# bonjour-l/esa-pose-estimation

Measured on AMD Instinct MI355X. Metric: HRNet-W32 256x256 crops/sec (heatmaps + fused argmax/refine keypoints), higher is better.
Workload: dtype bf16x6 (fp32-grade: every f32 operand split exactly into 3 bf16 terms, 6 bf16 MFMAs per product, f32 accumulate; f32 NHWC activations; f32 VALU stem conv1 / output layer) — heat-maps closer to fp64 than the fp32 CPU reference; 1 GPU; seg_hrnet2 HRNet-W32 256x256, batch 32/GPU, 11 keypoints, fp32 NCHW in -> heatmaps -> keypoints (BASELINE configs[1]); global_batch=32, per_gpu_batch=32, parallelism=dp1, hip_graph=True

## Files before the change

esa-pose-estimation_amd/csrc/forward.hip:

```cpp
#include <cstdarg>

#include "plan.h"

namespace esa {

__attribute__((format(printf, 3, 4)))
static void describe(esahrnet_op_desc* d, const char* kernel, const char* label, ...) {
    snprintf(d->kernel, sizeof d->kernel, "%s", kernel);
    va_list ap;
    va_start(ap, label);
    vsnprintf(d->label, sizeof d->label, label, ap);
    va_end(ap);
}

Request make_request(Decoder d, void* kp, void* idx, void* hess, void* fit, void* status, void* cov, void* info, double cov_floor,
                     int M, int nms_radius, int refine) {
    Request r;
    r.decoder = d;
    r.kp = static_cast<float*>(kp);
    r.idx = static_cast<int*>(idx);
    r.hess = d == DEC_FINAL ? nullptr : static_cast<double*>(hess);
    r.fit = static_cast<double*>(fit);
    r.status = static_cast<int*>(status);
    r.cov = d == DEC_GAUSSFIT || d == DEC_CAND ? static_cast<double*>(cov) : nullptr;
// ... 357 lines not shown
            p.x0 = T(o.in); p.y = T(o.out);
            p.w0 = static_cast<const uint4*>(c.head_w0); p.w3 = static_cast<const uint4*>(c.head_w3);
            p.bias0 = c.head_b0; p.bias3 = c.head_b3;
            p.N = n; p.H = lh[ti.level]; p.W = lw[ti.level];
            for (int i = 0; i < 3; ++i) {
                const Tensor& tt = c.tensors[o.terms[i]];
                p.t[i] = T(o.terms[i]); p.th[i] = lh[tt.level]; p.tw[i] = lw[tt.level];
                p.Ctp = tt.Cp;
            }
            p.C0p = ti.Cp; p.C3p = to.Cp; p.K = c.cfg.num_keypoints; p.valu = c.opt.bf_head_valu && !c.hf(); p.hf = c.hf();
            if (desc) {
                const ConvSpec& s0 = c.specs[c.spec_l0];
                const ConvSpec& s3 = c.specs[c.spec_l3];
                describe(desc, o.kind == OP_HEAD ? "head_fused" : c.x6() ? "head_x6" : c.hf() ? "head_fused_bf<fp16>" : "head_fused_bf",
                         "last_layer.0[:, 0:%d] + up + last_layer.3", c.head_c0);
                desc->flops = 2.0 * n * lh[to.level] * lw[to.level] * ((double)s0.cout * c.head_c0 + (double)s3.cout * s3.cin);
                desc->bytes = tbytes(o.in) + tbytes(o.out);
                for (int i = 0; i < 3; ++i) desc->bytes += tbytes(o.terms[i]);
            } else if (o.kind == OP_HEADBF) {
                rc = c.x6() ? esa::launch_head_x6(p, stream)
                   : b.h0_rec ? esa::launch_head_bf_range(p, b.h0_part, b.h0_rec, stream) : esa::launch_head_bf(p, stream);
            } else {
                if (!esa::head_fused_supported(p.H, p.W, p.th, p.tw, p.C0p, p.K))
                    return set_error("forward: fused head does not support this shape (%dx%d)", p.H, p.W);
                rc = esa::launch_head(p, stream);
            }
            break;
        }
        case OP_HEADT: {
            const Tensor& ti = c.tensors[o.in];
            const Tensor& to = c.tensors[o.out];
            const DevConv& d = c.dconvs[o.dconv];
            esa::HeadTParams p{};
            p.x = T(o.in); p.t = T(o.out); p.wt = static_cast<const uint4*>(d.w);
            p.N = n; p.h = lh[ti.level]; p.w = lw[ti.level];
            p.Cinp = ti.Cp; p.Ctp = to.Cp; p.XP = esa::head_t_xp(p.w);
            if (desc) {
                const ConvSpec& s = c.specs[d.spec];
                describe(desc, "head_t", "%s[:, %d:%d] (T layout)", s.name.c_str(), d.c0, d.c1);
                desc->flops = 2.0 * n * lh[ti.level] * lw[ti.level] * s.cout * (d.c1 - d.c0);
                desc->bytes = tbytes(o.in) + tbytes(o.out) + (double)esa::packed_weight_bytes(d.coutp, d.cinp, 1);
            } else rc = esa::launch_head_t(p, stream);
            break;
        }
        case OP_HEAD2: {
            const Tensor& ti = c.tensors[o.in];
            const Tensor& to = c.tensors[o.out];
            const DevConv& d1 = c.dconvs[o.dconv];
            esa::Head2Params p{};
            p.x0 = T(o.in); p.x1 = T(o.terms[0]); p.t2 = T(o.terms[1]); p.t3 = T(o.terms[2]); p.y = T(o.out);
            p.w0 = static_cast<const uint4*>(c.head_w0); p.w3 = static_cast<const uint4*>(c.head_w3);
            p.w1 = static_cast<const uint4*>(d1.w);
            p.bias0 = c.head_b0; p.bias3 = c.head_b3;
            p.N = n; p.H = lh[ti.level]; p.W = lw[ti.level];
            for (int i = 0; i < 3; ++i) {
                const Tensor& tt = c.tensors[o.terms[i]];
                p.th[i] = lh[tt.level]; p.tw[i] = lw[tt.level];
            }
            p.xp2 = esa::head_t_xp(p.tw[1]); p.xp3 = esa::head_t_xp(p.tw[2]);
            p.C0p = ti.Cp; p.C1p = c.tensors[o.terms[0]].Cp; p.Ctp = c.tensors[o.terms[1]].Cp;
            p.C3p = to.Cp; p.K = c.cfg.num_keypoints;
            if (desc) {
                const ConvSpec& s0 = c.specs[c.spec_l0];
                const ConvSpec& s3 = c.specs[c.spec_l3];
                const Tensor& t1 = c.tensors[o.terms[0]];
                describe(desc, "head_fused2", "last_layer.0[:, 0:%d] + up (MFMA) + last_layer.3", d1.c1);
                desc->flops = 2.0 * n * lh[to.level] * lw[to.level] * ((double)s0.cout * c.head_c0 + (double)s3.cout * s3.cin) +
                              2.0 * n * lh[t1.level] * lw[t1.level] * (double)s0.cout * (d1.c1 - d1.c0);
                desc->bytes = tbytes(o.in) + tbytes(o.out);
                for (int i = 0; i < 3; ++i) desc->bytes += tbytes(o.terms[i]);
            } else rc = esa::launch_head2(p, sp.head2_ulo, stream);
            break;
        }
        case OP_FUSE: {
            const Tensor& to = c.tensors[o.out];
            esa::FuseParams p{};
            p.nterms = o.nterms;
            for (int i = 0; i < o.nterms; ++i) {
                const Tensor& ti = c.tensors[o.terms[i]];
                if (ti.Cp != to.Cp) return set_error("plan bug: fuse channel mismatch");
                p.x[i] = T(o.terms[i]); p.h[i] = lh[ti.level]; p.w[i] = lw[ti.level];
            }
            p.y = T(o.out); p.N = n; p.H = lh[to.level]; p.W = lw[to.level]; p.Cp = to.Cp;
            p.relu = o.relu; p.fmt = c.opt.fmt;
            if (desc) {
                describe(desc, c.hf() ? "fuse_kernel<fp16>" : "fuse_kernel", "fuse -> %s", to.tap.c_str());
                desc->bytes = tbytes(o.out);
                for (int i = 0; i < o.nterms; ++i) desc->bytes += tbytes(o.terms[i]);
            } else rc = esa::launch_fuse(p, stream);
            break;
        }
        case OP_FINAL: {
            const Tensor& ti = c.tensors[o.in];
            esa::FinalParams p{};
            p.h3 = T(o.in); p.x0 = static_cast<const float*>(b.x); p.out = static_cast<float*>(b.heat);
            p.w = c.final_w; p.bias = c.final_b; p.wpk = static_cast<const uint4*>(c.final_wpk);
            p.N = n; p.H = height; p.W = width; p.h = lh[ti.level]; p.wd = lw[ti.level];
            p.K = c.cfg.num_keypoints; p.cin = c.cfg.cin; p.Cp = ti.Cp; p.fmt = c.opt.fmt;
            p.part = static_cast<float2*>(b.part);
            if (desc) {
                const ConvSpec& s = c.specs[c.spec_final];
                describe(desc, c.hf() ? "final_kernel<fp16>" : "final_kernel", "%s", s.name.c_str());
                desc->flops = 2.0 * n * height * width * s.cout * s.cin * 9;
                desc->bytes = tbytes(o.in) + (double)n * height * width * (c.cfg.cin + s.cout) * 4;
            } else if (b.req.decoder != DEC_NONE)
                rc = run_decode(c, b, &p, nullptr, 0, 0, n, height, width, stream);
            else rc = esa::launch_final(p, stream);
            break;
        }
    }
    if (rc) return set_error("forward: kernel launch failed: %s", hipGetErrorString((hipError_t)rc));
    return 0;
}

int run_forward(esahrnet_handle h, const void* x_dev, int n, int height, int width, void* heat_dev, void* part_dev, void* ws_dev,
                size_t ws_bytes, esahrnet_stream stream_, hipEvent_t* events, const Request* req, void* h0_part, void* h0_rec) {
    if (!h || !x_dev || !(heat_dev || req) || !ws_dev) return set_error("forward: null argument");
    if (!h->committed) return set_error("forward: esahrnet_commit has not been called");
    if (plan_shape(*h, n, height, width)) return 1;
    const KpScratch ks = kp_scratch(*h, n, height, width, req ? req->decoder : DEC_NONE, req ? req->refine : -1);
    if (check_workspace("forward", ws_dev, ws_bytes, h->sp.bytes + ks.total())) return 1;
    hipStream_t stream = static_cast<hipStream_t>(stream_);
    Buffers bufs{x_dev, heat_dev, static_cast<char*>(ws_dev), part_dev};
    bufs.h0_part = h0_part; bufs.h0_rec = h0_rec;
    if (req) {
        char* const scratch = bufs.ws + h->sp.bytes;
        bufs.req = *req;
        bufs.kheat = reinterpret_cast<float*>(scratch);
        bufs.kpart = reinterpret_cast<float2*>(scratch + ks.part_off());
        bufs.kbmax = reinterpret_cast<float*>(scratch + ks.bmax_off());
        bufs.kws = ks.part;
        bufs.kcidx = reinterpret_cast<int*>(scratch + ks.cidx_off());
        bufs.kat = scratch + ks.at_off();
    }
    int op_index = 0;
    if (events && hipEventRecord(events[0], stream) != hipSuccess) return set_error("forward: hipEventRecord failed");
    const bool multi = !events && !h->keep && h->opt.nlanes > 1 && h->side[0] != nullptr;
    const hipStream_t caller = stream;
    bool lane_used[4] = {true, false, false, false};
    int cur_wave = -1;
    auto join = [&](size_t slot, unsigned lanes) -> int {
        for (int l = 1; l < 4; ++l)
            if ((lanes >> l & 1) && lane_used[l]) {
                hipEvent_t e = h->wave_end[slot * 3 + l - 1];
                if (hipEventRecord(e, h->side[l - 1]) != hipSuccess || hipStreamWaitEvent(caller, e, 0) != hipSuccess) return 1;
                lane_used[l] = false;
            }
        return 0;
    };
    for (const Op& o : h->ops) {
        if (multi) {
            if (o.join && join((size_t)op_index, o.join)) return set_error("forward: joining side lanes failed");
            if (o.wave != cur_wave) {
                cur_wave = o.wave;
                if (h->wave_mask[cur_wave] & ~1u) HIP_OK(hipEventRecord(h->wave_entry[cur_wave], caller));
            }
            stream = o.lane == 0 ? caller : h->side[o.lane - 1];
            lane_used[o.lane] = true;
            if (o.wait_entry) HIP_OK(hipStreamWaitEvent(stream, h->wave_entry[cur_wave], 0));
            if (o.wait0 >= 0) HIP_OK(hipStreamWaitEvent(stream, h->op_event[o.wait0], 0));
        }
        if (run_op(*h, o, h->sp, bufs, stream, nullptr)) return 1;
        if (multi && o.record) HIP_OK(hipEventRecord(h->op_event[op_index], caller));
        ++op_index;
        if (events && hipEventRecord(events[op_index], stream) != hipSuccess) return set_error("forward: hipEventRecord failed");
    }
    if (multi && join(h->ops.size(), 0xeu)) return set_error("forward: joining the side lanes failed");
// ... 282 lines not shown
```

esa-pose-estimation_amd/csrc/fuse.hip:

```cpp
#include "kernels.h"
#include "sb.h"

namespace esa {
namespace {

static_assert(FMT_BF == EL_BF && FMT_HF == EL_HF && FMT_SB == EL_SB, "format codes double as element types");

struct Lerp {
    int i0, i1;
    float l0, l1;
};

__device__ __forceinline__ Lerp lerp_ac_false(int dst, int in, int out) {
    const float scale = (float)in / (float)out;
    float src = scale * ((float)dst + 0.5f) - 0.5f;
    src = src < 0.f ? 0.f : src;
    Lerp r;
    r.i0 = min((int)src, in - 1);
    r.i1 = r.i0 + (r.i0 < in - 1 ? 1 : 0);
    r.l1 = src - (float)r.i0;
    r.l0 = 1.f - r.l1;
    return r;
}

// ... 113 lines not shown
            load8<FMT_F32>(p.x[0] + ((row0 + (j >> 1)) * p.W + X + (j & 1)) * (size_t)pixb, c8, acc[j]);
    } else {
#pragma unroll
        for (int j = 0; j < 4; ++j)
#pragma unroll
            for (int i = 0; i < 8; ++i) acc[j][i] = 0.f;
    }
#pragma unroll
    for (int t = 1; t < NS; ++t)
#pragma unroll
        for (int j = 0; j < 4; ++j) {
            float v[8];
            load8<FMT_F32>(p.x[t] + ((row0 + (j >> 1)) * p.W + X + (j & 1)) * (size_t)pixb, c8, v);
#pragma unroll
            for (int i = 0; i < 8; ++i) acc[j][i] += v[i];
        }
#pragma unroll
    for (int k = 0; k < NU; ++k) {
        const int t = NS + k;
        const int h = p.h[t], w = p.w[t];
        const Lerp ly[2] = {lerp_scaled(Y, h, fs.sy[t]), lerp_scaled(Y + 1, h, fs.sy[t])};
        const Lerp lx[2] = {lerp_scaled(X, w, fs.sx[t]), lerp_scaled(X + 1, w, fs.sx[t])};
        const char* base = p.x[t] + (size_t)n * h * w * (size_t)pixb;
        const char* ra = base + (size_t)ly[0].i0 * w * (size_t)pixb;
        const char* rb = base + (size_t)ly[0].i1 * w * (size_t)pixb;
        const char* rc = base + (size_t)ly[1].i1 * w * (size_t)pixb;
        const int ca = lx[0].i0 * pixb, cb = lx[0].i1 * pixb, cc = lx[1].i1 * pixb;
        const bool sely = ly[1].i0 != ly[0].i0, selx = lx[1].i0 != lx[0].i0;
        const bool cell = (cell_mask >> t) & 1;
        if (cell) {
            float v00[8], v01[8], v10[8], v11[8];
            load8<FMT_F32>(ra + ca, c8, v00);
            load8<FMT_F32>(ra + cb, c8, v01);
            load8<FMT_F32>(rb + ca, c8, v10);
            load8<FMT_F32>(rb + cb, c8, v11);
#pragma unroll
            for (int j = 0; j < 4; ++j) {
                const int dy = j >> 1, dx = j & 1;
#pragma unroll
                for (int i = 0; i < 8; ++i)
                    acc[j][i] += ly[dy].l0 * (lx[dx].l0 * v00[i] + lx[dx].l1 * v01[i]) + ly[dy].l1 * (lx[dx].l0 * v10[i] + lx[dx].l1 * v11[i]);
            }
        } else {
            float v[3][3][8];
#pragma unroll
            for (int r = 0; r < 3; ++r) {
                const char* rr = r == 0 ? ra : r == 1 ? rb : rc;
                load8<FMT_F32>(rr + ca, c8, v[r][0]);
                load8<FMT_F32>(rr + cb, c8, v[r][1]);
                load8<FMT_F32>(rr + cc, c8, v[r][2]);
            }
#pragma unroll
            for (int i = 0; i < 8; ++i) {
                float c0[3][2], c1[3][2];
#pragma unroll
                for (int r = 0; r < 3; ++r) {
                    c0[r][0] = v[r][0][i]; c1[r][0] = v[r][1][i];
                    c0[r][1] = selx ? v[r][1][i] : v[r][0][i]; c1[r][1] = v[r][2][i];
                }
#pragma unroll
                for (int dx = 0; dx < 2; ++dx) {
                    const float a0 = lx[dx].l0 * c0[0][dx] + lx[dx].l1 * c1[0][dx];
                    const float b0 = lx[dx].l0 * c0[1][dx] + lx[dx].l1 * c1[1][dx];
                    const float g0 = lx[dx].l0 * c0[2][dx] + lx[dx].l1 * c1[2][dx];
                    acc[dx][i] += ly[0].l0 * a0 + ly[0].l1 * b0;
                    acc[2 + dx][i] += ly[1].l0 * (sely ? b0 : a0) + ly[1].l1 * g0;
                }
            }
        }
        __builtin_amdgcn_sched_barrier(0);
    }
#pragma unroll
    for (int j = 0; j < 4; ++j) {
        if (p.relu) {
#pragma unroll
            for (int i = 0; i < 8; ++i) acc[j][i] = relu1(acc[j][i]);
        }
        char* o = p.y + ((row0 + (j >> 1)) * p.W + X + (j & 1)) * (size_t)pixb + c8 * 32;
        *reinterpret_cast<f32x4*>(o) = f32x4{acc[j][0], acc[j][1], acc[j][2], acc[j][3]};
        *reinterpret_cast<f32x4*>(o + 16) = f32x4{acc[j][4], acc[j][5], acc[j][6], acc[j][7]};
    }
}

template <int NS, int NU>
int launch_fuse_t(const FuseParams& p, const FuseScales& fs, hipStream_t stream) {
    bool blocks = p.fmt == FMT_F32 && NU > 0 && !(p.H & 1) && !(p.W & 1);
    int cell_mask = 0;
    for (int t = NS; t < NS + NU && blocks; ++t) {
        if (2 * p.h[t] > p.H || 2 * p.w[t] > p.W) blocks = false;
        const bool exact = p.h[t] > 0 && p.w[t] > 0 && p.H % p.h[t] == 0 && p.W % p.w[t] == 0;
        const int ry = exact ? p.H / p.h[t] : 0, rx = exact ? p.W / p.w[t] : 0;
        if ((ry == 4 || ry == 8) && (rx == 4 || rx == 8)) cell_mask |= 1 << t;
    }
    if (blocks) {
        const long long per_row = (long long)(p.W >> 1) * (p.Cp >> 3), rows = (long long)p.N * (p.H >> 1);
        if (per_row <= 0 || rows <= 0 || rows > 0x7fffffffLL || per_row > 0x7fffffffLL) return (int)hipErrorInvalidValue;
        hipLaunchKernelGGL((fuse2x2_kernel<NS, NU>), dim3((unsigned)((per_row + 255) / 256), (unsigned)rows), dim3(256), 0, stream, p, fs, cell_mask);
        return (int)hipGetLastError();
    }
    const long long per_row = (long long)p.W * (p.Cp >> 3);
    const long long rows = (long long)p.N * p.H;
    if (per_row <= 0 || rows <= 0 || rows > 0x7fffffffLL || per_row > 0x7fffffffLL) return (int)hipErrorInvalidValue;
    const dim3 grid((unsigned)((per_row + 255) / 256), (unsigned)rows);
    if (p.fmt == FMT_BF) hipLaunchKernelGGL((fuse_kernel<NS, NU, FMT_BF>), grid, dim3(256), 0, stream, p, fs);
    else if (p.fmt == FMT_HF) hipLaunchKernelGGL((fuse_kernel<NS, NU, FMT_HF>), grid, dim3(256), 0, stream, p, fs);
    else if (p.fmt == FMT_F32) hipLaunchKernelGGL((fuse_kernel<NS, NU, FMT_F32>), grid, dim3(256), 0, stream, p, fs);
    else hipLaunchKernelGGL((fuse_kernel<NS, NU, FMT_SB>), grid, dim3(256), 0, stream, p, fs);
    return (int)hipGetLastError();
}

}

int launch_fuse(const FuseParams& p_in, hipStream_t stream) {
    if ((p_in.Cp & 7) || p_in.nterms < 1 || p_in.nterms > 4) return (int)hipErrorInvalidValue;
    FuseParams p = p_in;
    FuseScales fs{};
    int ns = 0, k = 0;
    for (int pass = 0; pass < 2; ++pass)
        for (int t = 0; t < p_in.nterms; ++t) {
            const bool same = p_in.h[t] == p_in.H && p_in.w[t] == p_in.W;
            if (same != (pass == 0)) continue;
            p.x[k] = p_in.x[t]; p.h[k] = p_in.h[t]; p.w[k] = p_in.w[t];
            fs.sy[k] = (float)p_in.h[t] / (float)p_in.H;
            fs.sx[k] = (float)p_in.w[t] / (float)p_in.W;
            ++k;
            if (same) ++ns;
        }
    const int nu = p.nterms - ns;
    switch (ns * 10 + nu) {
        case 1: return launch_fuse_t<0, 1>(p, fs, stream);
        case 2: return launch_fuse_t<0, 2>(p, fs, stream);
        case 3: return launch_fuse_t<0, 3>(p, fs, stream);
        case 4: return launch_fuse_t<0, 4>(p, fs, stream);
        case 10: return launch_fuse_t<1, 0>(p, fs, stream);
        case 11: return launch_fuse_t<1, 1>(p, fs, stream);
        case 12: return launch_fuse_t<1, 2>(p, fs, stream);
        case 13: return launch_fuse_t<1, 3>(p, fs, stream);
        case 20: return launch_fuse_t<2, 0>(p, fs, stream);
        case 21: return launch_fuse_t<2, 1>(p, fs, stream);
        case 22: return launch_fuse_t<2, 2>(p, fs, stream);
        case 30: return launch_fuse_t<3, 0>(p, fs, stream);
        case 31: return launch_fuse_t<3, 1>(p, fs, stream);
        case 40: return launch_fuse_t<4, 0>(p, fs, stream);
    }
    return (int)hipErrorInvalidValue;
}

}
```

esa-pose-estimation_amd/csrc/kernels.h:

```cpp
#pragma once
#include <hip/hip_runtime.h>
#include <stdint.h>

namespace esa {

enum { FMT_SB = 0, FMT_BF = 1, FMT_F32 = 2, FMT_HF = 3 };
inline bool fmt_half(int fmt) { return fmt == FMT_BF || fmt == FMT_HF; }

int set_error(const char* fmt, ...);

struct ConvParams {
    const char* x;
    char* y;
    const char* res;
    const uint4* w;
    const float* bias;
    int N, H, W, OH, OW;
    int Cinp, Coutp;
    int relu;
    int out_f32;
    int fmt;
    int nheads;
    int x6_reload;
    char* yh[3];
// ... 2 lines not shown
};
bool conv_s2c32_multi_supported(const ConvParams& p);
int launch_conv_s2c32_multi(const ConvParams& p, hipStream_t stream);
int launch_conv(const ConvParams& p, int k, int stride, hipStream_t stream);
const char* conv_kernel_name(const ConvParams& p, int k, int stride);
bool conv_s2c32_supported(const ConvParams& p);
int launch_conv_s2c32(const ConvParams& p, hipStream_t stream);
int launch_conv_s1w(const ConvParams& p, hipStream_t stream);
bool conv_is_stream_s1(const ConvParams& p);
bool conv_jobs_supported(const ConvParams* ps, int n, int stride);
int launch_conv_jobs(const ConvParams* ps, int n, int stride, hipStream_t stream);
bool use_th16(const ConvParams& p);
void set_stream_launch_limit(long long bytes);
bool conv1x1_supported(const ConvParams& p);
int launch_conv1x1(const ConvParams& p, hipStream_t stream);
bool conv1x1_jobs_supported(const ConvParams* ps, int n);
int launch_conv1x1_jobs(const ConvParams* ps, int n, hipStream_t stream);
size_t packed_weight_bytes(int coutp, int cinp, int k);
void pack_conv_weights(const float* w, int cout, int cin, int k, int coutp, int cinp, void* dst);
size_t packed_weight_bytes_bf(int coutp, int cinp, int k);
void pack_conv_weights_bf(const float* w, int cout, int cin, int k, int coutp, int cinp, void* dst, bool half = false);
uint16_t host_f16(float f);
bool host_f16_finite(float f);

size_t packed_weight_bytes_x6(int coutp, int cinp, int k);
void pack_conv_weights_x6(const float* w, int cout, int cin, int k, int coutp, int cinp, void* dst);
bool conv_x6_supported(const ConvParams& p, int k, int stride);
int launch_conv_x6(const ConvParams& p, int k, int stride, hipStream_t stream);
const char* conv_x6_kernel_name(const ConvParams& p, int k, int stride);
bool conv_x6_jobs_supported(const ConvParams* ps, int n, int k, int stride);
int launch_conv_x6_jobs(const ConvParams* ps, int n, int k, int stride, hipStream_t stream);
void set_x6_grid_limit(int workgroups);
bool conv1x1_x6_supported(const ConvParams& p);
int launch_conv1x1_x6(const ConvParams& p, hipStream_t stream);
int launch_conv1x1_x6_jobs(const ConvParams* ps, int n, hipStream_t stream);
bool conv1x1_x6_jobs_supported(const ConvParams* ps, int n);

struct StemParams {
    const float* x;
    char* y;
    const float* w;
    const float* bias;
    int N, H, W, cin, cout;
    int relu;
    int fmt;
};
int launch_stem(const StemParams& p, hipStream_t stream);
int stem_pool_slabs(int cin, int cout, int H, int W);
int launch_stem_pool(const StemParams& p, float* pool, hipStream_t stream);

struct BlockParams {
    const char* x;
    char* y;
    const uint4* w1;
    const uint4* w2;
    const float* bias1;
    const float* bias2;
    int N, H, W;
};
int launch_bblock32(const BlockParams& p, hipStream_t stream);

struct StemFusedParams {
    const float* x;
    char* y;
    const float* w1;
    const float* bias1;
    const uint4* w2;
    const float* bias2;
    int N, H, W, OH, OW, cin, Cmid, Coutp;
};
int launch_stem_fused(const StemFusedParams& p, hipStream_t stream);
bool stem_fused_x6_supported(int cin, int cmid, int coutp);
void pack_stem_w1_x6(const float* w, const float* b, float* dst);
int launch_stem_fused_x6(const StemFusedParams& p, hipStream_t stream);

struct FuseParams {
    const char* x[4];
    int h[4], w[4];
    int nterms;
    char* y;
    int N, H, W, Cp;
    int relu;
    int fmt;
};
int launch_fuse(const FuseParams& p, hipStream_t stream);

struct FinalParams {
    const char* h3;
    const float* x0;
    float* out;
    const float* w;
    const float* bias;
    const uint4* wpk;
    int N, H, W, h, wd;
    int K, cin, Cp;
    int fmt;
    float2* part;
};
int launch_final(const FinalParams& p, hipStream_t stream);
int final_kp_tiles(int K, int cin, int H, int W);
int launch_final_kp(const FinalParams& p, float* kp, int* idx_out, hipStream_t stream);
int launch_final_gf(const FinalParams& p, float* kp, int* idx_out, double* fit, int* status, double* hess, hipStream_t stream);
int launch_final_gf_cov(const FinalParams& p, float* kp, int* idx_out, double* fit, int* status, double* hess, double* cov,
                        double* info, double cov_floor, hipStream_t stream);
int final2_valu_tiles(int H, int W);
int launch_final2_kp(const FinalParams& p, float* bmax, float* kp, int* idx_out, hipStream_t stream, double* hess = nullptr);
int final_part_tiles(int K, int cin, int H, int W);
__device__ __forceinline__ void argmax_take(float v, int i, float& bv, int& bi) {
    const bool vn = v != v, bn = bv != bv;
    if (v > bv || (vn && !bn) || ((v == bv || (vn && bn)) && i < bi)) { bv = v; bi = i; }
}
bool final_mfma_supported(int K, int cin);
size_t final_mfma_bytes(int K, int cin);
void pack_final_mfma(const float* w, int K, int cin, void* dst);

struct HeadParams {
    const char* x0;
    const char* t[3];
    char* y;
    const uint4* w0;
    const uint4* w3;
    const float* bias0;
    const float* bias3;
    int N, H, W;
    int th[3], tw[3];
    int C0p, Ctp, C3p, K;
    bool valu;
    bool hf;
};
int launch_head(const HeadParams& p, hipStream_t stream);
bool head_fused_supported(int H, int W, const int th[3], const int tw[3], int C0p, int K);
size_t head_w3_bytes(int K, int Ctp);
void pack_head_w3(const float* w, int K, int Ct, int Ctp, void* dst);
int launch_head_bf(const HeadParams& p, hipStream_t stream);
bool head_fused_bf_supported(int H, int W, const int th[3], const int tw[3], int C0p, int K);
int head_bf_range_tiles(int H, int W);
int launch_head_bf_range(const HeadParams& p, void* part, void* rec, hipStream_t stream);
size_t head_w3_bf_bytes(int K, int Ctp);
void pack_head_w3_bf(const float* w, int K, int Ct, int Ctp, void* dst, bool half = false);

int launch_head_x6(const HeadParams& p, hipStream_t stream);
bool head_x6_supported(int H, int W, const int th[3], const int tw[3], int C0p, int K);

constexpr int HT_PAD = 1;
struct HeadTParams {
    const char* x;
    char* t;
    const uint4* wt;
    int N, h, w, Cinp, Ctp, XP;
};
int launch_head_t(const HeadTParams& p, hipStream_t stream);
int head_t_xp(int w);
bool head_t_supported(int Cinp);
struct Head2Params {
    const char* x0;
    const char* x1;
    const char* t2;
    const char* t3;
    char* y;
    const uint4* w0;
    const uint4* w1;
    const uint4* w3;
    const float* bias0;
    const float* bias3;
    int N, H, W;
    int th[3], tw[3];
// ... 157 lines not shown
```

esa-pose-estimation_amd/csrc/op_abi.hip:

```cpp
#include <algorithm>
#include <cstdint>
#include <cstdio>
#include <cstring>
#include <vector>

#include "../../include/esahrnet.h"
#include "host_util.h"
#include "kernels.h"

using esa::DevScope;
using esa::Format;
using esa::set_error;

static const float* f32(const void* p) { return static_cast<const float*>(p); }
static float* f32(void* p) { return static_cast<float*>(p); }
static bool aligned(const void* p, uintptr_t a) { return (reinterpret_cast<uintptr_t>(p) & (a - 1)) == 0; }

static bool conv_form_ok(int k, int stride) { return (k == 1 && stride == 1) || (k == 3 && (stride == 1 || stride == 2)); }
static bool op_conv_dims_ok(int n, int cin, int cout, int h, int w, int k, int stride) {
    if (n <= 0 || cin <= 0 || cout <= 0 || h <= 0 || w <= 0 || !conv_form_ok(k, stride)) return false;
    return (long long)n * h * w * (long long)((std::max(cin, cout) + 63) & ~63) * 4 <= 0x7fffffffLL;
}
static esa::ConvParams op_conv_shape(const Format& f, int n, int cin, int cout, int h, int w, int stride, int relu, const void* res) {
    esa::ConvParams p{};
    p.N = n; p.H = h; p.W = w; p.OH = stride == 2 ? (h + 1) / 2 : h; p.OW = stride == 2 ? (w + 1) / 2 : w;
    p.Cinp = f.pad(cin); p.Coutp = f.pad(cout); p.relu = relu; p.fmt = f.fmt;
    p.res = static_cast<const char*>(res);
    p.x6_reload = esa::env_on("ESAHRNET_X6_RELOAD_WEIGHTS");
    return p;
}
static int op_conv_device(DevScope& m, const Format& f, esa::ConvParams& p, int cin, int cout, int k, const float* w, const float* b,
                          const void* x_dev, const void* res_dev, int* rc) {
    std::vector<float> bias(p.Coutp, 0.f);
    std::copy(b, b + cout, bias.begin());
    char *xs = nullptr, *rs = nullptr;
    if (m.upload(f.pack(w, cout, cin, k, p.Coutp, p.Cinp), &p.w) || m.upload(bias, &p.bias)) return 1;
    const size_t xb = (size_t)p.N * p.H * p.W * p.Cinp * f.eb, yb = (size_t)p.N * p.OH * p.OW * p.Coutp * f.eb;
    if (m.alloc(&xs, xb) || m.alloc(&p.y, yb) || (res_dev && m.alloc(&rs, yb))) return 1;
    *rc = esa::launch_nchw_to_fmt(f.fmt, f32(x_dev), p.N, cin, p.H, p.W, xs, p.Cinp, m.stream());
    if (!*rc && res_dev) *rc = esa::launch_nchw_to_fmt(f.fmt, f32(res_dev), p.N, cout, p.OH, p.OW, rs, p.Coutp, m.stream());
    p.x = xs; p.res = rs;
    return 0;
}

extern "C" {

int esahrnet_op_conv(const void* x_dev, int n, int cin, int height, int width, const float* w,
                     const float* b, int cout, int k, int stride, int relu, const void* res_dev,
                     void* y_dev, esahrnet_stream stream_) {
    return esahrnet_op_conv_ex(x_dev, n, cin, height, width, w, b, cout, k, stride, relu, res_dev, y_dev, 0, stream_);
}

int esahrnet_op_conv_ex(const void* x_dev, int n, int cin, int height, int width, const float* w,
                        const float* b, int cout, int k, int stride, int relu, const void* res_dev,
                        void* y_dev, int precision, esahrnet_stream stream_) {
    if (!x_dev || !w || !b || !y_dev) return set_error("op_conv: null argument");
    if (precision < 0 || precision > 3) return set_error("op_conv: precision %d", precision);
    if (!conv_form_ok(k, stride)) return set_error("op_conv: k=%d stride=%d unsupported", k, stride);
    const Format f(precision);
    DevScope m("op_conv", static_cast<hipStream_t>(stream_));
    esa::ConvParams p = op_conv_shape(f, n, cin, cout, height, width, stride, relu, res_dev);
    int rc = 0;
    if (op_conv_device(m, f, p, cin, cout, k, w, b, x_dev, res_dev, &rc)) return 1;
    if (!rc) rc = esa::launch_conv(p, k, stride, m.stream());
    if (!rc) rc = esa::launch_fmt_to_nchw(f.fmt, p.y, n, cout, p.OH, p.OW, p.Coutp, f32(y_dev), m.stream());
    return m.finish(rc);
}

int esahrnet_op_fuse(const void* const* xs_dev, const int* hs, const int* ws, int nterms, int n, int c,
                     int height, int width, int relu, void* y_dev, esahrnet_stream stream_) {
    return esahrnet_op_fuse_ex(xs_dev, hs, ws, nterms, n, c, height, width, relu, y_dev, 0, stream_);
}

int esahrnet_op_fuse_ex(const void* const* xs_dev, const int* hs, const int* ws, int nterms, int n, int c,
                        int height, int width, int relu, void* y_dev, int precision, esahrnet_stream stream_) {
    if (!xs_dev || !hs || !ws || !y_dev || nterms < 1 || nterms > 4) return set_error("op_fuse: bad argument");
    if (precision < 0 || precision > 3) return set_error("op_fuse: precision %d", precision);
    const Format f(precision);
    DevScope m("op_fuse", static_cast<hipStream_t>(stream_));
    const int cp = f.pad(c);
    int rc = 0;
    esa::FuseParams p{};
    p.nterms = nterms; p.N = n; p.H = height; p.W = width; p.Cp = cp; p.relu = relu; p.fmt = f.fmt;
    for (int i = 0; i < nterms && !rc; ++i) {
        char* x = nullptr;
        if (m.alloc(&x, (size_t)n * hs[i] * ws[i] * cp * f.eb)) return 1;
        rc = esa::launch_nchw_to_fmt(f.fmt, f32(xs_dev[i]), n, c, hs[i], ws[i], x, cp, m.stream());
        p.x[i] = x; p.h[i] = hs[i]; p.w[i] = ws[i];
    }
    if (!rc && m.alloc(&p.y, (size_t)n * height * width * cp * f.eb)) return 1;
    if (!rc) rc = esa::launch_fuse(p, m.stream());
    if (!rc) rc = esa::launch_fmt_to_nchw(f.fmt, p.y, n, c, height, width, cp, f32(y_dev), m.stream());
    return m.finish(rc);
}

int esahrnet_op_cbam(const void* x_dev, const void* res_dev, int n, int c, int height, int width, const float* w_fc0,
                     const float* w_fc2, const float* w_sa, int relu, void* y_dev, int cy, int c0, int fused, int precision,
                     esahrnet_stream stream_) {
    return esahrnet_op_cbam_steps(x_dev, res_dev, n, c, height, width, w_fc0, w_fc2, w_sa, relu, y_dev, cy, c0, fused, precision,
                                  0, nullptr, nullptr, nullptr, stream_);
}

int esahrnet_op_cbam_steps(const void* x_dev, const void* res_dev, int n, int c, int height, int width, const float* w_fc0,
                           const float* w_fc2, const float* w_sa, int relu, void* y_dev, int cy, int c0, int fused, int precision,
                           int slabs, void* partial_out, void* ca_out, void* maps_out, esahrnet_stream stream_) {
    if (!x_dev || !w_fc0 || !w_fc2 || !w_sa || !y_dev || n <= 0 || height <= 0 || width <= 0) return set_error("op_cbam: bad argument");
    if (precision < 0 || precision > 2) return set_error("op_cbam: precision %d", precision);
    if (c < 16 || (c & 7)) return set_error("op_cbam: c=%d (a multiple of 8, at least 16: ChannelAttention's ratio)", c);
    const Format f(precision);
    const int cp = f.pad(c), cyp = f.pad(cy);
    if (cp > 512) return set_error("op_cbam: c=%d is %d channels padded, ca_mlp serves at most 512", c, cp);
    if (c0 < 0 || (c0 & 7) || c0 + cp > cyp) return set_error("op_cbam: slice [%d, %d) outside the %d channels of y", c0, c0 + cp, cyp);
    if (fused && !esa::cbam_spatial_supported(cp)) return set_error("op_cbam: cbam_spatial does not serve %d channels", cp);
    if (fused && maps_out) return set_error("op_cbam: maps_out with fused = 1 (cbam_spatial keeps the maps in LDS)");
    if ((long long)height * width > 0x7fffffffLL / n) return set_error("op_cbam: %d x %d x %d pixels", n, height, width);
    const int cr = c / 16, hw = height * width;
    if (slabs < 0 || slabs > std::min(1024, hw)) return set_error("op_cbam: slabs=%d (0, or 1 .. min(1024, %d pixels))", slabs, hw);
    const int P = slabs ? slabs : std::min(esa::POOL_SLABS, hw);
    DevScope m("op_cbam", static_cast<hipStream_t>(stream_));
    hipStream_t stream = m.stream();
    const std::vector<float> h0(w_fc0, w_fc0 + (size_t)cr * c), h2(w_fc2, w_fc2 + (size_t)c * cr), hs(w_sa, w_sa + 98);
    char *xs = nullptr, *rs = nullptr, *ys = nullptr;
    float *part = nullptr, *ca = nullptr, *maps = nullptr, *w0 = nullptr, *w2 = nullptr, *wsa = nullptr;
    if (m.upload(h0, &w0) || m.upload(h2, &w2) || m.upload(hs, &wsa)) return 1;
    const size_t npix = (size_t)n * hw;
    const size_t part_bytes = (size_t)n * P * cp * 2 * sizeof(float), ca_bytes = (size_t)n * cp * sizeof(float),
                 maps_bytes = npix * 2 * sizeof(float);
    if (m.alloc(&xs, npix * cp * f.eb) || (res_dev && m.alloc(&rs, npix * cp * f.eb)) || m.alloc(&ys, npix * cyp * f.eb) ||
        m.alloc(&part, part_bytes) || m.alloc(&ca, ca_bytes) || m.alloc(&maps, maps_bytes)) return 1;
    int rc = esa::launch_nchw_to_fmt(f.fmt, f32(x_dev), n, c, height, width, xs, cp, stream);
    if (!rc && res_dev) rc = esa::launch_nchw_to_fmt(f.fmt, f32(res_dev), n, c, height, width, rs, cp, stream);
    if (!rc) rc = esa::launch_nchw_to_fmt(f.fmt, f32(y_dev), n, cy, height, width, ys, cyp, stream);
    if (!rc) rc = esa::launch_pool_partial(xs, part, n, hw, cp, P, stream, f.fmt);
    if (!rc) rc = esa::launch_ca_mlp(part, w0, w2, ca, n, hw, c, cp, cr, P, stream);
    esa::CbamApplyParams ap{};
    ap.x = xs; ap.res = rs; ap.ca = ca; ap.maps = maps; ap.w_sa = wsa; ap.y = ys;
    ap.N = n; ap.H = height; ap.W = width; ap.Cp = cp; ap.y_pix_bytes = cyp * f.eb; ap.y_c0 = c0; ap.relu = relu; ap.C = c; ap.fmt = f.fmt;
    if (!rc && fused) rc = esa::launch_cbam_spatial(ap, stream);
    if (!rc && !fused) rc = esa::launch_cbam_maps(ap.x, ap.ca, maps, n, hw, c, cp, stream, f.fmt);
    if (!rc && !fused) rc = esa::launch_cbam_apply(ap, stream);
    if (!rc) rc = esa::launch_fmt_to_nchw(f.fmt, ys, n, cy, height, width, cyp, f32(y_dev), stream);
    hipError_t ce = hipSuccess;
    if (!rc && partial_out) ce = hipMemcpyAsync(partial_out, part, part_bytes, hipMemcpyDeviceToDevice, stream);
    if (!rc && ce == hipSuccess && ca_out) ce = hipMemcpyAsync(ca_out, ca, ca_bytes, hipMemcpyDeviceToDevice, stream);
    if (!rc && ce == hipSuccess && maps_out) ce = hipMemcpyAsync(maps_out, maps, maps_bytes, hipMemcpyDeviceToDevice, stream);
    return m.finish(rc, ce, "copying a step's output");
}

int esahrnet_op_stem(const void* x_dev, int n, int height, int width, const float* w, const float* b, int relu, int pooled,
                     int precision, void* y_dev, void* partial_out, int* slabs_out, esahrnet_stream stream_) {
    if (!x_dev || !w || !b || !y_dev || n <= 0 || height <= 0 || width <= 0) return set_error("op_stem: bad argument");
    if (precision < 0 || precision > 2) return set_error("op_stem: precision %d (0, 1 or 2)", precision);
    if ((long long)height * width > 0x7fffffffLL / 64 / n) return set_error("op_stem: %d x %d x %d pixels", n, height, width);
    constexpr int cout = 64;
    const int slabs = pooled ? esa::stem_pool_slabs(1, cout, height, width) : 0;
    if (pooled && (!partial_out || !slabs_out)) return set_error("op_stem: pooled = 1 needs partial_out and slabs_out");
    if (pooled && slabs <= 0) return set_error("op_stem: launch_stem_pool does not serve %d x %d", height, width);
    const Format f(precision);
    DevScope m("op_stem", static_cast<hipStream_t>(stream_));
    const std::vector<float> wp = esa::pack_stem_w(w, cout, 1, cout), bp(b, b + cout);
    const float *dw = nullptr, *db = nullptr;
    char* ys = nullptr;
    float* part = nullptr;
    if (m.upload(wp, &dw) || m.upload(bp, &db)) return 1;
    const size_t part_bytes = (size_t)n * slabs * cout * 2 * sizeof(float);
    if (m.alloc(&ys, (size_t)n * height * width * cout * f.eb) || (pooled && m.alloc(&part, part_bytes))) return 1;
// ... 263 lines not shown
```

esa-pose-estimation_amd/csrc/plan.h:

```cpp
#pragma once
#include <algorithm>
#include <cmath>
#include <cstdio>
#include <cstring>
#include <map>
#include <string>
#include <vector>

#include "../../include/esahrnet.h"
#include "host_util.h"

#pragma GCC visibility push(hidden)
namespace esa {

struct ConvSpec {
    std::string name, bn;
    int cin, cout, k, stride, level;
    bool has_bias, relu;
    std::vector<float> w, b;
    bool set = false;
    int parent = -1, pc0 = 0, pc1 = 0;
};

struct DevConv {
// ... 4 lines not shown
    std::vector<int> perm;
    int cinp, coutp;
    void* w = nullptr;
    float* bias = nullptr;
};

enum OpKind { OP_STEM, OP_STEMF, OP_CONV, OP_BLOCK, OP_FUSE, OP_HEAD, OP_HEADT, OP_HEAD2, OP_FINAL, OP_HEADBF,
              OP_STEMRAW, OP_POOL, OP_MLP, OP_MAPS, OP_APPLY, OP_RESAMPLE, OP_ZERO, OP_TONCHW, OP_GATHER };

struct AuxSpec {
    std::string name;
    int shape[4];
    std::vector<float> data;
    bool set = false;
    float* dev = nullptr;
};

struct Tensor {
    int C, Cp, level;
    int flat = 0;
    std::string tap;
    std::string key;
    bool tlayout = false;
    bool f32 = false;
    int alt = 0;
    int def = -1, last = -1;
    size_t off = 0;
};

struct Op {
    OpKind kind;
    int dconv = -1;
    int dconv2 = -1;
    int in = -1, out = -1, res = -1;
    int out2 = -1;
    int terms[4] = {-1, -1, -1, -1};
    int nterms = 0;
    bool relu = false;
    int lane = 0;
    int wave = 0;
    int wait0 = -1;
    bool wait_entry = false;
    bool record = false;
    unsigned join = 0;
    int aux[3] = {-1, -1, -1};
    int c0 = 0;
    int nchan = 0;
    int align = 0;
    int alt = 0;
    int multi = -1, mpos = 0;
    int jkey = -1;
    int job = -1, jpos = 0;
};

struct Multi {
    int n = 0;
    int op[3] = {-1, -1, -1};
    void* w = nullptr;
    float* bias = nullptr;
    int coutp = 0;
};

struct JobGroup {
    int n = 0;
    int op[6] = {-1, -1, -1, -1, -1, -1};
};

struct ShapePlan {
    int n = 0, h = 0, w = 0;
    bool keep = false;
    size_t bytes = 0;
    std::vector<int> lh, lw;
    bool head2 = false;
    bool head2_ulo = false;
    std::vector<char> multi_on;
    std::vector<char> job_on;
};

enum StemForm { STEM_SEPARATE, STEM_FUSED, STEM_FUSED_X6 };
enum HeadForm { HEAD_UNFUSED, HEAD_SB, HEAD_BF, HEAD_X6 };

struct PlanOptions {
    bool unfused, head_v1, final_valu, no_multihead, no_jobs, no_bblock, no_cbam_jobs, cbam_unfused, stem_pool_separate,
         head3_direct, head3_cout32, bf_unfused_head, bf_head_valu, x6_unfused_head, x6_unfused_stem, x6_reload_weights, tap_all;
    int nlanes;
    int fmt;
    StemForm stem;
    bool fused_block;
    HeadForm head;
    bool head2;
    bool final_mfma;
};

struct ScaleRange { int c0, c1, group; };

enum Decoder { DEC_NONE, DEC_FINAL, DEC_FINAL2, DEC_GAUSSFIT, DEC_CAND };
struct Request {
    Decoder decoder = DEC_NONE;
    float* kp = nullptr;
    int* idx = nullptr;
    double* hess = nullptr;
    double* fit = nullptr;
    int* status = nullptr;
    double* cov = nullptr;
    double* info = nullptr;
    double cov_floor = 0.0;
    float* cand = nullptr;
    int* cidx = nullptr;
    int M = 0, r = 0;
    int refine = -1;
};

struct Buffers {
    const void* x;
    void* heat;
    char* ws;
    void* part;
    Request req;
    float* kheat = nullptr;
    float2* kpart = nullptr;
    float* kbmax = nullptr;
    size_t kws = 0;
    int* kcidx = nullptr;
    void* kat = nullptr;
    void* h0_part = nullptr;
    void* h0_rec = nullptr;
};

}

struct esahrnet_ctx {
    esahrnet_cfg cfg;
    int device;
    std::vector<esa::ConvSpec> specs;
    std::map<std::string, int> spec_by_name;
    std::vector<esa::DevConv> dconvs;
    std::vector<esa::AuxSpec> aux;
    float *stemraw_w = nullptr, *stemraw_b = nullptr;
    std::vector<esa::Tensor> tensors;
    std::vector<esa::Op> ops;
    int spec_stem = -1, spec_final = -1;
    float *stem_w = nullptr, *stem_b = nullptr, *final_w = nullptr, *final_b = nullptr;
    void* final_wpk = nullptr;
    int spec_l0 = -1, spec_l3 = -1, head_c0 = 0;
    void *head_w0 = nullptr, *head_w3 = nullptr;
    float *head_b0 = nullptr, *head_b3 = nullptr;
    bool committed = false;
    bool keep = false;
    esa::PlanOptions opt;
    esa::Format format;
    bool h16() const { return format.half; }
    bool hf() const { return format.hf; }
    bool x6() const { return format.x6; }
    int padc(int ch) const { return format.pad(ch); }
    int eb() const { return format.eb; }
    size_t wbytes(int coutp, int cinp, int k) const { return format.wbytes(coutp, cinp, k); }
    std::vector<char> pack(const float* w, int cout, int cin, int k, int coutp, int cinp) const { return format.pack(w, cout, cin, k, coutp, cinp); }
    int head2_op = -1;
    int nwaves = 1;
    std::vector<int> wave_last;
    std::vector<unsigned char> wave_mask;
    hipStream_t side[3] = {nullptr, nullptr, nullptr};
    std::vector<hipEvent_t> wave_entry;
    std::vector<hipEvent_t> wave_end;
    std::vector<hipEvent_t> op_event;
    esa::ShapePlan sp;
    int max_level = 0;
// ... 52 lines not shown
```

esa-pose-estimation_amd/csrc/plan_build.hip:

```cpp
#include "plan.h"

namespace esa {

PlanOptions plan_options(const esahrnet_cfg& g, const esa::Format& format) {
    const auto on = esa::env_on;
    PlanOptions o;
    o.unfused = on("ESAHRNET_UNFUSED"); o.head_v1 = on("ESAHRNET_HEAD_V1"); o.final_valu = on("ESAHRNET_FINAL_VALU");
    o.no_multihead = on("ESAHRNET_NO_MULTIHEAD"); o.no_jobs = on("ESAHRNET_NO_JOBS"); o.no_bblock = on("ESAHRNET_NO_BBLOCK");
    o.no_cbam_jobs = on("ESAHRNET_NO_CBAM_JOBS"); o.cbam_unfused = on("ESAHRNET_CBAM_UNFUSED");
    o.stem_pool_separate = on("ESAHRNET_STEM_POOL_SEPARATE"); o.head3_direct = on("ESAHRNET_HEAD3_DIRECT");
    o.head3_cout32 = on("ESAHRNET_HEAD3_COUT32"); o.bf_unfused_head = on("ESAHRNET_BF_UNFUSED_HEAD");
    o.bf_head_valu = on("ESAHRNET_BF_HEAD_VALU"); o.x6_unfused_head = on("ESAHRNET_X6_UNFUSED_HEAD");
    o.x6_unfused_stem = on("ESAHRNET_X6_UNFUSED_STEM"); o.tap_all = on("ESAHRNET_TAP_ALL");
    o.x6_reload_weights = on("ESAHRNET_X6_RELOAD_WEIGHTS");
    const char* streams = getenv("ESAHRNET_STREAMS");
    o.nlanes = streams && atoi(streams) > 1 ? 4 : 1;
    o.fmt = format.fmt;
    const bool sb = o.fmt == esa::FMT_SB, v0 = g.variant == 0;
    const bool x6_stem = esa::stem_fused_x6_supported(g.cin, pad32(g.stem_width), pad32(g.stem_width)) && g.stem_width == 64;
    o.stem = sb && (!v0 || !o.unfused) ? STEM_FUSED
           : o.fmt == esa::FMT_F32 && x6_stem && !o.x6_unfused_stem ? STEM_FUSED_X6 : STEM_SEPARATE;
    o.fused_block = sb && v0 && !o.unfused && !o.no_bblock;
    int nb4 = 0;
    while (nb4 < ESAHRNET_MAX_BRANCHES && g.blocks[3][nb4] > 0) ++nb4;
    const int c0 = pad32(g.widths[0]);
    o.head = !v0 || nb4 != 4 ? HEAD_UNFUSED
           : sb ? (!o.unfused && (c0 == 32 || c0 == 64) ? HEAD_SB : HEAD_UNFUSED)
           : esa::fmt_half(o.fmt) ? (!o.bf_unfused_head && (pad64(g.widths[0]) == 64 || pad64(g.widths[0]) == 128) ? HEAD_BF : HEAD_UNFUSED)
           : !o.x6_unfused_head && (c0 == 32 || c0 == 64) ? HEAD_X6 : HEAD_UNFUSED;
    o.head2 = !o.head_v1 && (o.head != HEAD_SB || ((pad32(g.widths[1]) == 64 || pad32(g.widths[1]) == 96) &&
                                                   esa::head_t_supported(pad32(g.widths[2])) && esa::head_t_supported(pad32(g.widths[3]))));
    o.final_mfma = v0 && o.fmt != esa::FMT_F32 && !o.final_valu && esa::final_mfma_supported(g.num_keypoints, g.cin);
    return o;
}

namespace {

struct Builder {
    esahrnet_ctx& c;
    int jkey = -1;
    int jkey2 = -1;
    explicit Builder(esahrnet_ctx& ctx) : c(ctx) {}

    int spec(const std::string& name, const std::string& bn, int cin, int cout, int k, int stride,
             int level, bool bias, bool relu) {
        ConvSpec s;
        s.name = name; s.bn = bn; s.cin = cin; s.cout = cout; s.k = k; s.stride = stride;
        s.level = level; s.has_bias = bias; s.relu = relu;
        c.specs.push_back(s);
        c.spec_by_name[name] = (int)c.specs.size() - 1;
        c.max_level = std::max(c.max_level, level);
        return (int)c.specs.size() - 1;
    }
    int taps_spec(int parent, int c0, int c1, int level) {
        const std::string name = c.specs[parent].name + "#taps[" + std::to_string(c0) + ":" + std::to_string(c1) + "]";
        const int cout9 = 9 * ((c.specs[parent].cout + 7) & ~7);
        const int sp = spec(name, "", c1 - c0, cout9, 1, 1, level, false, false);
        c.specs[sp].parent = parent; c.specs[sp].pc0 = c0; c.specs[sp].pc1 = c1;
        if (c.nhost_specs < 0) c.nhost_specs = sp;
        return sp;
    }
    int tensor(int C, int level, const std::string& tap = "") {
        Tensor t;
        t.C = C; t.Cp = c.padc(C); t.level = level; t.tap = tap; t.key = tap;
        c.tensors.push_back(t);
        return (int)c.tensors.size() - 1;
    }
    void use(int t, int op) {
        if (t < 0) return;
        c.tensors[t].last = std::max(c.tensors[t].last, op);
    }
    int conv(int sp, int in, int res, bool relu, const std::string& tap = "", int c0 = 0, int c1 = -1,
             bool use_bias = true, bool out_f32 = false) {
        const ConvSpec& s = c.specs[sp];
        DevConv d;
        d.spec = sp; d.c0 = c0; d.c1 = c1 < 0 ? s.cin : c1; d.use_bias = use_bias; d.out_f32 = out_f32;
        d.cinp = c.padc(d.c1 - d.c0); d.coutp = c.padc(s.cout);
        c.dconvs.push_back(d);
        Op o;
        o.kind = OP_CONV; o.dconv = (int)c.dconvs.size() - 1; o.in = in; o.res = res; o.relu = relu;
        if (jkey >= 0 && s.k == 3 && s.stride == 1) o.jkey = jkey++;
        if (jkey2 >= 0 && ((s.k == 3 && s.stride == 2) || s.k == 1)) o.jkey = jkey2;
        o.out = tensor(s.cout, s.level, tap.empty() && !out_f32 && c.opt.tap_all ? "conv:" + s.name : tap);
        c.tensors[o.out].f32 = out_f32;
        c.tensors[o.out].key = !tap.empty() ? tap : d.c0 != 0 || d.c1 != s.cin
            ? s.name + "[:, " + std::to_string(d.c0) + ":" + std::to_string(d.c1) + "]" : s.name;
        const int idx = (int)c.ops.size();
        c.tensors[o.out].def = idx;
        use(in, idx); use(res, idx);
        c.ops.push_back(o);
        return o.out;
    }
    int fuse(const std::vector<int>& terms, int C, int level, bool relu, const std::string& tap = "", const std::string& key = "") {
        Op o;
        o.kind = OP_FUSE; o.nterms = (int)terms.size(); o.relu = relu;
        o.out = tensor(C, level, tap);
        if (tap.empty()) c.tensors[o.out].key = key;
// ... 681 lines not shown
```

Before: 8281 crops/s.

## Add 4-channel-per-thread 2x2 fuse kernel with grouped upsample loads

Adds a new fuse2x2 quad kernel for the f32 path in which each thread handles 4 channels instead of 8 over a 2x2 output block. Upsample-term loads are split into register-budgeted groups at compile time, with asm pins and sched barriers to bound live registers, and the cell mask is specialised as a template parameter. The aim is to cut register pressure, raise occupancy and memory parallelism in the HRNet fuse layers, and drop runtime branching on the cell mask. The trade-offs are twice as many threads, more template instantiations, and some loss of vector width per thread. The old kernel stays reachable through an env flag.

```diff
diff --git a/esa-pose-estimation_amd/csrc/forward.hip b/esa-pose-estimation_amd/csrc/forward.hip
--- a/esa-pose-estimation_amd/csrc/forward.hip
+++ b/esa-pose-estimation_amd/csrc/forward.hip
@@ -463,7 +463,7 @@
                 p.x[i] = T(o.terms[i]); p.h[i] = lh[ti.level]; p.w[i] = lw[ti.level];
             }
             p.y = T(o.out); p.N = n; p.H = lh[to.level]; p.W = lw[to.level]; p.Cp = to.Cp;
-            p.relu = o.relu; p.fmt = c.opt.fmt;
+            p.relu = o.relu; p.fmt = c.opt.fmt; p.fuse2x2_v1 = c.opt.fuse2x2_v1;
             if (desc) {
                 describe(desc, c.hf() ? "fuse_kernel<fp16>" : "fuse_kernel", "fuse -> %s", to.tap.c_str());
                 desc->bytes = tbytes(o.out);
diff --git a/esa-pose-estimation_amd/csrc/fuse.hip b/esa-pose-estimation_amd/csrc/fuse.hip
--- a/esa-pose-estimation_amd/csrc/fuse.hip
+++ b/esa-pose-estimation_amd/csrc/fuse.hip
@@ -219,6 +219,168 @@
     }
 }
 
+constexpr int kQuadBudget = 72;
+constexpr int quad_groups(int ns, int nu, int cells) {
+    int used = ns > 1 ? 16 * (ns - 1) : 0, g = 0, packed = 0;
+    for (int k = 0; k < nu; ++k) {
+        const int need = (cells >> k) & 1 ? 16 : 36;
+        if (used > 0 && used + need > kQuadBudget) { ++g; used = 0; }
+        used += need;
+        packed |= g << (2 * k);
+    }
+    return packed;
+}
+
+__device__ __forceinline__ f32x4 load4(const char* row, unsigned off) { return *reinterpret_cast<const f32x4*>(row + off); }
+__device__ __forceinline__ void pin(unsigned& a) { asm volatile("" : "+v"(a)); }
+__device__ __forceinline__ void pin(int& a) { asm volatile("" : "+v"(a)); }
+__device__ __forceinline__ void pin(float& a) { asm volatile("" : "+v"(a)); }
+
+template <int NS, int NU, int CELLS>
+__global__ __launch_bounds__(256) void fuse2x2_quad_kernel(FuseParams p, FuseScales fs) {
+    constexpr int GROUPS = quad_groups(NS, NU, CELLS), NG = ((GROUPS >> (2 * (NU - 1))) & 3) + 1;
+    const int Q = p.Cp >> 2, W2 = p.W >> 1, H2 = p.H >> 1;
+    const unsigned u = blockIdx.x * 256u + threadIdx.x;
+    if (u >= (unsigned)(W2 * Q)) return;
+    const int bx = (int)(u / (unsigned)Q);
+    const int c4 = (int)(u - (unsigned)bx * (unsigned)Q);
+    const int brow = blockIdx.y;
+    const int n = brow / H2, by = brow - n * H2;
+    const int X = 2 * bx, Y = 2 * by;
+    const int pixb = p.Cp * 4;
+    const size_t row0 = (size_t)n * p.H + Y;
+    const size_t rowb = (size_t)p.W * (size_t)pixb;
+    unsigned o0 = (unsigned)(X * pixb + c4 * 16), o1 = o0 + (unsigned)pixb;
+
+    Lerp ly[NU][2], lx[NU][2];
+    const char *ra[NU], *rb[NU], *rc[NU];
+    unsigned ca[NU], cb[NU], cc[NU];
+    bool sely[NU];
+    int selx[NU];
+#pragma unroll
+    for (int k = 0; k < NU; ++k) {
+        const int t = NS + k;
+        const int h = p.h[t], w = p.w[t];
+        ly[k][0] = lerp_scaled(Y, h, fs.sy[t]); ly[k][1] = lerp_scaled(Y + 1, h, fs.sy[t]);
+        lx[k][0] = lerp_scaled(X, w, fs.sx[t]); lx[k][1] = lerp_scaled(X + 1, w, fs.sx[t]);
+        const char* base = p.x[t] + (size_t)n * h * w * (size_t)pixb;
+        ra[k] = base + (size_t)ly[k][0].i0 * w * (size_t)pixb;
+        rb[k] = base + (size_t)ly[k][0].i1 * w * (size_t)pixb;
+        rc[k] = base + (size_t)ly[k][1].i1 * w * (size_t)pixb;
+        ca[k] = (unsigned)(lx[k][0].i0 * pixb + c4 * 16);
+        cb[k] = (unsigned)(lx[k][0].i1 * pixb + c4 * 16);
+        cc[k] = (unsigned)(lx[k][1].i1 * pixb + c4 * 16);
+        sely[k] = ly[k][1].i0 != ly[k][0].i0; selx[k] = lx[k][1].i0 != lx[k][0].i0;
+    }
+
+    f32x4 acc[4];
+    f32x4 s[NS > 1 ? NS - 1 : 1][4];
+    f32x4 v[NU][3][3];
+#pragma unroll
+    for (int g = 0; g < NG; ++g) {
+        if (g == 0) { pin(o0); pin(o1); }
+#pragma unroll
+        for (int k = 0; k < NU; ++k) {
+            if (((GROUPS >> (2 * k)) & 3) != g) continue;
+            pin(ca[k]); pin(cb[k]);
+            if (!((CELLS >> k) & 1)) pin(cc[k]);
+        }
+        __builtin_amdgcn_sched_barrier(0);
+        if (g == 0) {
+#pragma unroll
+            for (int t = 0; t < NS; ++t)
+#pragma unroll
+                for (int j = 0; j < 4; ++j) {
+                    const f32x4 x = load4(p.x[t] + (row0 + (j >> 1)) * rowb, (j & 1) ? o1 : o0);
+                    if (t == 0) acc[j] = x;
+                    else s[t > 0 ? t - 1 : 0][j] = x;
+                }
+        }
+#pragma unroll
+        for (int k = 0; k < NU; ++k) {
+            if (((GROUPS >> (2 * k)) & 3) != g) continue;
+            const bool cell = (CELLS >> k) & 1;
+#pragma unroll
+            for (int r = 0; r < 3; ++r) {
+                if (cell && r == 2) continue;
+                const char* rr = r == 0 ? ra[k] : r == 1 ? rb[k] : rc[k];
+                v[k][r][0] = load4(rr, ca[k]);
+                v[k][r][1] = load4(rr, cb[k]);
+                if (!cell) v[k][r][2] = load4(rr, cc[k]);
+            }
+        }
+        __builtin_amdgcn_sched_barrier(0);
+        if (g == 0) {
+            if (NS == 0) {
+#pragma unroll
+                for (int j = 0; j < 4; ++j) acc[j] = f32x4{0.f, 0.f, 0.f, 0.f};
+            }
+#pragma unroll
+            for (int t = 1; t < NS; ++t)
+#pragma unroll
+                for (int j = 0; j < 4; ++j)
+#pragma unroll
+                    for (int i = 0; i < 4; ++i) acc[j][i] += s[t - 1][j][i];
+        }
+#pragma unroll
+        for (int k = 0; k < NU; ++k) {
+            if (((GROUPS >> (2 * k)) & 3) != g) continue;
+            Lerp* lyk = ly[k];
+            Lerp* lxk = lx[k];
+#pragma unroll
+            for (int d = 0; d < 2; ++d) { pin(lxk[d].l0); pin(lxk[d].l1); }
+            if (!((CELLS >> k) & 1)) pin(selx[k]);
+            if ((CELLS >> k) & 1) {
+#pragma unroll
+                for (int j = 0; j < 4; ++j) {
+                    const int dy = j >> 1, dx = j & 1;
+#pragma unroll
+                    for (int i = 0; i < 4; ++i)
+                        acc[j][i] += lyk[dy].l0 * (lxk[dx].l0 * v[k][0][0][i] + lxk[dx].l1 * v[k][0][1][i]) +
+                                     lyk[dy].l1 * (lxk[dx].l0 * v[k][1][0][i] + lxk[dx].l1 * v[k][1][1][i]);
+                }
+            } else {
+#pragma unroll
+                for (int i = 0; i < 4; ++i) {
+                    float c0[3][2], c1[3][2];
+#pragma unroll
+                    for (int r = 0; r < 3; ++r) {
+                        c0[r][0] = v[k][r][0][i]; c1[r][0] = v[k][r][1][i];
+                        c0[r][1] = selx[k] ? v[k][r][1][i] : v[k][r][0][i]; c1[r][1] = v[k][r][2][i];
+                    }
+#pragma unroll
+                    for (int dx = 0; dx < 2; ++dx) {
+                        const float a0 = lxk[dx].l0 * c0[0][dx] + lxk[dx].l1 * c1[0][dx];
+                        const float b0 = lxk[dx].l0 * c0[1][dx] + lxk[dx].l1 * c1[1][dx];
+                        const float g0 = lxk[dx].l0 * c0[2][dx] + lxk[dx].l1 * c1[2][dx];
+                        acc[dx][i] += lyk[0].l0 * a0 + lyk[0].l1 * b0;
+                        acc[2 + dx][i] += lyk[1].l0 * (sely[k] ? b0 : a0) + lyk[1].l1 * g0;
+                    }
+                }
+            }
+        }
+        if (g + 1 < NG) __builtin_amdgcn_sched_barrier(0);
+    }
+#pragma unroll
+    for (int j = 0; j < 4; ++j) {
+        if (p.relu) {
+#pragma unroll
+            for (int i = 0; i < 4; ++i) acc[j][i] = relu1(acc[j][i]);
+        }
+        *reinterpret_cast<f32x4*>(p.y + (row0 + (j >> 1)) * rowb + ((j & 1) ? o1 : o0)) = acc[j];
+    }
+}
+
+template <int NS, int NU, int CELLS = (1 << NU) - 1>
+int launch_quad(const FuseParams& p, const FuseScales& fs, int cells, dim3 grid, hipStream_t stream) {
+    if (cells == CELLS) {
+        hipLaunchKernelGGL((fuse2x2_quad_kernel<NS, NU, CELLS>), grid, dim3(256), 0, stream, p, fs);
+        return (int)hipGetLastError();
+    }
+    if constexpr (CELLS > 0) return launch_quad<NS, NU, CELLS - 1>(p, fs, cells, grid, stream);
+    return (int)hipErrorInvalidValue;
+}
+
 template <int NS, int NU>
 int launch_fuse_t(const FuseParams& p, const FuseScales& fs, hipStream_t stream) {
     bool blocks = p.fmt == FMT_F32 && NU > 0 && !(p.H & 1) && !(p.W & 1);
@@ -230,9 +392,15 @@
         if ((ry == 4 || ry == 8) && (rx == 4 || rx == 8)) cell_mask |= 1 << t;
     }
     if (blocks) {
-        const long long per_row = (long long)(p.W >> 1) * (p.Cp >> 3), rows = (long long)p.N * (p.H >> 1);
+        const long long rows = (long long)p.N * (p.H >> 1);
+        const bool quad = !p.fuse2x2_v1 && (long long)p.W * p.Cp * 4 <= 0x7fffffffLL;
+        const long long per_row = (long long)(p.W >> 1) * (quad ? p.Cp >> 2 : p.Cp >> 3);
         if (per_row <= 0 || rows <= 0 || rows > 0x7fffffffLL || per_row > 0x7fffffffLL) return (int)hipErrorInvalidValue;
-        hipLaunchKernelGGL((fuse2x2_kernel<NS, NU>), dim3((unsigned)((per_row + 255) / 256), (unsigned)rows), dim3(256), 0, stream, p, fs, cell_mask);
+        const dim3 grid((unsigned)((per_row + 255) / 256), (unsigned)rows);
+        if constexpr (NU > 0) {
+            if (quad) return launch_quad<NS, NU>(p, fs, cell_mask >> NS, grid, stream);
+        }
+        hipLaunchKernelGGL((fuse2x2_kernel<NS, NU>), grid, dim3(256), 0, stream, p, fs, cell_mask);
         return (int)hipGetLastError();
     }
     const long long per_row = (long long)p.W * (p.Cp >> 3);
diff --git a/esa-pose-estimation_amd/csrc/kernels.h b/esa-pose-estimation_amd/csrc/kernels.h
--- a/esa-pose-estimation_amd/csrc/kernels.h
+++ b/esa-pose-estimation_amd/csrc/kernels.h
@@ -108,6 +108,7 @@
     int N, H, W, Cp;
     int relu;
     int fmt;
+    int fuse2x2_v1;
 };
 int launch_fuse(const FuseParams& p, hipStream_t stream);
 
diff --git a/esa-pose-estimation_amd/csrc/op_abi.hip b/esa-pose-estimation_amd/csrc/op_abi.hip
--- a/esa-pose-estimation_amd/csrc/op_abi.hip
+++ b/esa-pose-estimation_amd/csrc/op_abi.hip
@@ -82,6 +82,7 @@
     int rc = 0;
     esa::FuseParams p{};
     p.nterms = nterms; p.N = n; p.H = height; p.W = width; p.Cp = cp; p.relu = relu; p.fmt = f.fmt;
+    p.fuse2x2_v1 = esa::env_on("ESAHRNET_FUSE2X2_V1");
     for (int i = 0; i < nterms && !rc; ++i) {
         char* x = nullptr;
         if (m.alloc(&x, (size_t)n * hs[i] * ws[i] * cp * f.eb)) return 1;
diff --git a/esa-pose-estimation_amd/csrc/plan.h b/esa-pose-estimation_amd/csrc/plan.h
--- a/esa-pose-estimation_amd/csrc/plan.h
+++ b/esa-pose-estimation_amd/csrc/plan.h
@@ -110,7 +110,7 @@
 
 struct PlanOptions {
     bool unfused, head_v1, final_valu, no_multihead, no_jobs, no_bblock, no_cbam_jobs, cbam_unfused, stem_pool_separate,
-         head3_direct, head3_cout32, bf_unfused_head, bf_head_valu, x6_unfused_head, x6_unfused_stem, x6_reload_weights, tap_all;
+         head3_direct, head3_cout32, bf_unfused_head, bf_head_valu, x6_unfused_head, x6_unfused_stem, x6_reload_weights, fuse2x2_v1, tap_all;
     int nlanes;
     int fmt;
     StemForm stem;
diff --git a/esa-pose-estimation_amd/csrc/plan_build.hip b/esa-pose-estimation_amd/csrc/plan_build.hip
--- a/esa-pose-estimation_amd/csrc/plan_build.hip
+++ b/esa-pose-estimation_amd/csrc/plan_build.hip
@@ -13,6 +13,7 @@
     o.bf_head_valu = on("ESAHRNET_BF_HEAD_VALU"); o.x6_unfused_head = on("ESAHRNET_X6_UNFUSED_HEAD");
     o.x6_unfused_stem = on("ESAHRNET_X6_UNFUSED_STEM"); o.tap_all = on("ESAHRNET_TAP_ALL");
     o.x6_reload_weights = on("ESAHRNET_X6_RELOAD_WEIGHTS");
+    o.fuse2x2_v1 = on("ESAHRNET_FUSE2X2_V1");
     const char* streams = getenv("ESAHRNET_STREAMS");
     o.nlanes = streams && atoi(streams) > 1 ? 4 : 1;
     o.fmt = format.fmt;
```

New measurement: 8301 crops/s (median of 6 runs). No clear change (+0.2%).
